# hahnicity/deepards

Measured on AMD Instinct MI355X. Metric: breath-sequences/sec (train step) cnn_linear nb20 seq224, higher is better.
Workload: dtype f32; 1 GPU; cnn_linear+resnet18, synthetic (B=64 per GPU, 20, 1, 224) fp32 train step (BASELINE configs[1]); backbone=resnet18, batch_per_gpu=64, global_batch=64, batch_rule=--batch 64 per rank (weak scaling: the global batch grows with the ranks), n_sub_batches=20, seq_len=224, optimizer=sgd-nesterov+clamp, parallelism=dp1, hipgraph=True

## Files before the change

deepards_amd/csrc/common.h:

```cpp
#pragma once
#include <hip/hip_runtime.h>
#include <stdint.h>

typedef float f32x4 __attribute__((ext_vector_type(4)));
typedef float f32x16 __attribute__((ext_vector_type(16)));

typedef float f32x2v __attribute__((ext_vector_type(2)));
typedef __bf16 bf16x2v __attribute__((ext_vector_type(2)));

#define DA_OK 0
#define DA_EINVAL (-1)

__device__ __forceinline__ int xcd_chunked(int id, int total) {
  const int q = total >> 3, r = total & 7;
  const int xcd = id & 7, s = id >> 3;
  return (xcd < r ? xcd * (q + 1) : r * (q + 1) + (xcd - r) * q) + s;
}

__device__ __forceinline__ uint32_t mix32(uint32_t a, uint32_t b) {
  uint32_t h = a * 0x9E3779B1u ^ (b + 0x7F4A7C15u);
  h ^= h >> 16; h *= 0x85EBCA6Bu;
  h ^= h >> 13; h *= 0xC2B2AE35u;
  h ^= h >> 16;
  return h;
// ... 349 lines not shown
static inline int wgrad_pre_grid(WgradPreTable& pre, int blocks, bool front = false) {
  if (pre.nblocks == 0) return blocks;
  pre.own = front ? -1 : (blocks + 7) & ~7;
  return (front ? blocks : pre.own) + pre.nblocks;
}

struct WgradChain {
  WgradPreTable pre, next;
  int pre_job[WGRAD_PRE_MAX], next_job[WGRAD_PRE_MAX];
  float* const* dws;
  int* reduced;
};
static inline void wgrad_chain_init(WgradChain* c, float* const* dws, int accumulate, int* reduced) {
  c->pre.n = c->pre.nblocks = c->pre.own = 0;
  c->pre.first_block[0] = 0;
  c->pre.accumulate = accumulate;
  c->next = c->pre;
  c->dws = dws;
  c->reduced = reduced;
}
static inline void wgrad_chain_offer(WgradChain* c, int job, const da_wgrad_job& j, int splits) {
  if (!c || !c->dws || !c->dws[job] || c->next.n >= WGRAD_PRE_MAX) return;
  WgradPreTable& t = c->next;
  t.d[t.n] = {j.workspace, c->dws[job], splits, j.ntaps, j.N, j.C};
  c->next_job[t.n] = job;
  t.first_block[t.n + 1] = t.first_block[t.n] + (j.ntaps * j.N * j.C + 1023) / 1024;
  ++t.n;
  t.nblocks = (t.first_block[t.n] + 7) & ~7;
}
static inline WgradPreTable wgrad_chain_take(WgradChain* c) {
  WgradPreTable t;
  t.n = t.nblocks = t.accumulate = t.own = 0;
  t.first_block[0] = 0;
  if (!c) return t;
  t = c->pre;
  for (int i = 0; i < t.n; ++i) c->reduced[c->pre_job[i]] = 1;
  c->pre = c->next;
  for (int i = 0; i < c->next.n; ++i) c->pre_job[i] = c->next_job[i];
  c->next.n = c->next.nblocks = 0;
  return t;
}

struct WgradPlan {
  int tn, tc;
  int splits;
  int kchunk;
};
int wgrad_plan_jobs(const da_wgrad_job* jobs, int n, int chained, WgradPlan* plan);

bool wino_wgrad_eligible(const da_wgrad_job& j);
void wino_wgrad_plan_jobs(const da_wgrad_job* jobs, int n, int chained, WgradPlan* plan);
int wino_wgrad_launch(const da_wgrad_job* jobs, const WgradPlan* plan, int n, hipStream_t stream, WgradChain* chain);
void wino4_wgrad_plan(int rows, int L, int* splits, int* qchunk);
int wino4_wgrad_launch(const da_wgrad_job* jobs, const WgradPlan* plan, int n, hipStream_t stream, WgradChain* chain);

bool bf16_wgrad_eligible(const da_wgrad_job& j);
void bf16_wgrad_plan(int rows, int L, int* splits, int* pchunk);
int bf16_wgrad_launch(const da_wgrad_job* jobs, const WgradPlan* plan, int n, int code, hipStream_t stream);

typedef struct {
  const float* x;
  const float* w;
  float* y;
  int rows, Lm, Lsrc, ldx, C, Ldst, ldy, N, dst_stride, dst_off, src_stride, ntaps;
  int src_off[3];
  int wtap[3];
  int accumulate;
  const float* x2;
  const float* w2;
  int tap_split;
} da_conv_job;

extern "C" int da_sizeof_wgrad_reduce_desc(void);
extern "C" int da_sizeof_bn_running_desc(void);
extern "C" int da_sizeof_bn_pgrad_desc(void);
```

deepards_amd/csrc/conv_gemm.hip:

```cpp
#include "common.h"
#include <algorithm>
#include <utility>
#include <vector>

#ifndef WGRAD_GLOAD_AT
#define WGRAD_GLOAD_AT 8
#endif
#ifndef GLOAD_AT
#define GLOAD_AT 3
#endif

struct ConvGemmArgs {
  const float* x;
  const float* w;
  const float* x2;
  const float* w2;
  int tap_split;
  float* y;
  int M, Lsrc, ldx, C;
  int Ldst, ldy, N;
  int dst_stride, dst_off, src_stride;
  int ntaps, so0, so1, so2, wt0, wt1, wt2;
  int accumulate;
  FastDiv divLm;
// ... 1111 lines not shown
  int n_xf = 0;
  for (int i = 0; i < n; ++i) {
    const da_wgrad_job& j = jobs[i];
    if (!j.dy || !j.x || j.ntaps < 1 || j.ntaps > 3 || j.C % 32 || j.N % 32 || j.lddy % 4 || j.ldx % 4 ||
        (j.winograd == 49 && (j.lddy != j.N || j.ldx != j.C)))
      return DA_EINVAL;
    if ((uint64_t)j.rows * j.Lm * (uint64_t)j.Lm >= 0xffffffffull) return DA_EINVAL;
    if (j.winograd != 0 && j.winograd != 1 && j.winograd != 6 && j.winograd != 16 && j.winograd != 49) return DA_EINVAL;
    if ((j.xform || j.dy_half) && (j.winograd || j.src_stride != 1 || j.dy_stride != 1 || j.dy_off || j.Lm != j.Lx ||
                                   (j.dy_half && j.ntaps != 1)))
      return DA_EINVAL;
    if (j.dy_half && !j.xform) return DA_EINVAL;
    if (j.xform && (j.xform != 1 || !j.mean || !j.invstd || !j.gamma || !j.beta || j.Wn < 1 || j.ldstat < j.C || j.ldstat % 4 ||
                    j.Wn < 32 || (uint64_t)j.rows * j.Lm * (uint64_t)j.Wn >= 0xffffffffull))
      return DA_EINVAL;
    if (j.dy_half && (j.Lm & 1 || j.Ldy * 2 != j.Lm)) return DA_EINVAL;
    if (g_act_bf16 && j.winograd != 16) return DA_EINVAL;
    if (j.winograd == 16 || j.winograd == 49 ? !bf16_wgrad_eligible(j) : (j.winograd && !wino_wgrad_eligible(j))) return DA_EINVAL;
    n_xf += (j.xform || j.dy_half) ? 1 : 0;
  }
  const int tgt = (chained && g_wgrad_any && n_xf >= 8) ? (2560 / n_xf < 96 ? 96 : 2560 / n_xf) : 0;
  for (int i = 0; i < n; ++i) {
    const da_wgrad_job& j = jobs[i];
    plan[i].tn = plan[i].tc = 64;
    if (j.winograd == 16 || j.winograd == 49) bf16_wgrad_plan(j.rows, j.Lm, &plan[i].splits, &plan[i].kchunk);
    else if (j.winograd == 6) wino4_wgrad_plan(j.rows, j.Lm, &plan[i].splits, &plan[i].kchunk);
    else if (j.winograd == 0) {
      plan[i] = wgrad_plan(j.rows * j.Lm, j.N, j.C, j.ntaps, (j.xform || j.dy_half) ? tgt : 0);
      if (!plan[i].tn) return DA_EINVAL;
    }
  }
  wino_wgrad_plan_jobs(jobs, n, chained, plan);
  return DA_OK;
}

static void conv_gemm_fill(ConvGemmArgs& g, const da_conv_job& j) {
  g.x = j.x; g.w = j.w; g.y = j.y;
  g.x2 = j.x2 ? j.x2 : j.x; g.w2 = j.w2 ? j.w2 : j.w; g.tap_split = j.x2 ? j.tap_split : 3;
  g.M = j.rows * j.Lm; g.Lsrc = j.Lsrc; g.ldx = j.ldx; g.C = j.C;
  g.Ldst = j.Ldst; g.ldy = j.ldy; g.N = j.N;
  g.dst_stride = j.dst_stride; g.dst_off = j.dst_off; g.src_stride = j.src_stride;
  g.ntaps = j.ntaps;
  g.so0 = j.src_off[0]; g.so1 = j.ntaps > 1 ? j.src_off[1] : 0; g.so2 = j.ntaps > 2 ? j.src_off[2] : 0;
  g.wt0 = j.wtap[0]; g.wt1 = j.ntaps > 1 ? j.wtap[1] : 0; g.wt2 = j.ntaps > 2 ? j.wtap[2] : 0;
  g.accumulate = j.accumulate;
  g.divLm = make_fastdiv((uint32_t)j.Lm);
}

extern "C" {

int da_debug_set(int key, int value) {
  if (key == 3) g_use_tail = value;
  else if (key == 7) g_wgrad_any = value;
  else return DA_EINVAL;
  return DA_OK;
}

int da_conv_gemm(const float* x, const float* w, float* y, int rows, int Lm, int Lsrc, int ldx, int C, int Ldst,
                 int ldy, int N, int dst_stride, int dst_off, int src_stride, int ntaps, const int* src_off,
                 const int* wtap, int accumulate, hipStream_t stream) {
  DA_ENTER();
  if (g_act_bf16) return DA_EINVAL;
  if (!x || !w || !y || rows < 0 || Lm < 1 || ntaps < 1 || ntaps > 3) return DA_EINVAL;
  da_conv_job j = {};
  j.x = x; j.w = w; j.y = y;
  j.rows = rows; j.Lm = Lm; j.Lsrc = Lsrc; j.ldx = ldx; j.C = C; j.Ldst = Ldst; j.ldy = ldy; j.N = N;
  j.dst_stride = dst_stride; j.dst_off = dst_off; j.src_stride = src_stride; j.ntaps = ntaps; j.accumulate = accumulate;
  for (int t = 0; t < ntaps; ++t) {
    j.src_off[t] = src_off[t];
    j.wtap[t] = wtap[t];
  }
  ConvGemmArgs a;
  conv_gemm_fill(a, j);
  return conv_gemm_dispatch(a, stream);
}

int da_conv_gemm_multi(const da_conv_job* jobs, int n, hipStream_t stream) {
  DA_ENTER();
  if (g_act_bf16) return DA_EINVAL;
  if (n < 1 || n > 4 || !jobs) return DA_EINVAL;
  ConvGemmArgs a[4];
  for (int i = 0; i < n; ++i) {
    const da_conv_job& j = jobs[i];
    if (!j.x || !j.w || !j.y || j.rows < 0 || j.Lm < 1 || j.ntaps < 1 || j.ntaps > 3 || j.C % 32 || j.N % 64 || j.ldx % 4)
      return DA_EINVAL;
    if ((uint64_t)j.rows * j.Lm * (uint64_t)j.Lm >= 0xffffffffull) return DA_EINVAL;
    if (j.x2 && (!j.w2 || j.tap_split < 1 || j.tap_split >= j.ntaps)) return DA_EINVAL;
    conv_gemm_fill(a[i], j);
  }
  return launch_conv_multi(a, n, stream);
}

int da_conv1x1_bn(const float* x, int ldx, const float* w, float* y, int ldy, int rows, int R, int Lin, int C, int N, int pool,
                  float* mean, float* invstd, int ldstat, const float* gamma, const float* beta, const float* pend, int pend_c0,
                  long pend_units, int pend_Wu, float eps, float* out_part, hipStream_t stream) {
  DA_ENTER();
  if (g_act_bf16) return DA_EINVAL;
  if (!x || !w || !y || !mean || !invstd || !gamma || !beta || rows < 0 || R < 1 || rows % R || Lin < 1) return DA_EINVAL;
  if (C % 32 || C < 32 || C > 2048 || N % 64 || N < 64 || ldx % 4 || ldx < C || ldy < N || ldstat % 4 || ldstat < C) return DA_EINVAL;
  if (pool && (Lin & 1)) return DA_EINVAL;
  if (rows == 0) return DA_OK;
  const int Lout = pool ? Lin / 2 : Lin;
  const long M = (long)rows * Lout;
  if ((long)R * Lout < 64) return DA_EINVAL;
  if ((uint64_t)rows * Lin * (uint64_t)(ldx > ldy ? ldx : ldy) >= 0x7fffffffull) return DA_EINVAL;
  if ((uint64_t)M * (uint64_t)(R * Lout) >= 0xffffffffull) return DA_EINVAL;
// ... 233 lines not shown
```

deepards_amd/csrc/conv_wino.hip:

```cpp
#include "common.h"
#include <type_traits>

struct WinoArgs {
  const float* x;
  const float* u;
  float* y;
  int MP, L, PL, ldx, C, ldy, N, accumulate;
  FastDiv divPL;
  const long long* drop_seed;
  uint32_t drop_salt;
  float drop_p;
  float* stat_part;
  int stat_Wu;
  const float* in_pend;
  float* in_mean;
  float* in_invstd;
  const float* in_gamma;
  const float* in_beta;
  int in_tiles, in_Wu;
  float in_eps;
};

__device__ __forceinline__ int wino_row(int i) {
  return (i >= 4 && i < 12) ? 2 * (i - 4) : (i < 4 ? 2 * i + 1 : 2 * (i - 12) + 9);
// ... 444 lines not shown
        }
    }
  }

  if (MINI) {
    __syncthreads();
    f32x4* red = reinterpret_cast<f32x4*>(lds);
    if (khalf == 1) {
#pragma unroll
      for (int j = 0; j < 6; ++j)
#pragma unroll
        for (int nt = 0; nt < 2; ++nt) red[((wp * 6 + j) * 2 + nt) * 64 + lane] = acc[j][nt];
    }
    __syncthreads();
    if (khalf == 1) return;
#pragma unroll
    for (int j = 0; j < 6; ++j)
#pragma unroll
      for (int nt = 0; nt < 2; ++nt) {
        const f32x4 o = red[((wp * 6 + j) * 2 + nt) * 64 + lane];
#pragma unroll
        for (int e = 0; e < 4; ++e) acc[j][nt][e] += o[e];
      }
  }

#pragma unroll
  for (int r = 0; r < 4; ++r) {
    const int Q = Q0 + wp * 16 + wino_row(g * 4 + r);
    if (Q >= a.MP) continue;
    const uint32_t rr = fdiv((uint32_t)Q, a.divPL);
    const int i = Q - (int)rr * QL;
    const int nvalid = a.L - 4 * i;
    float* yp = a.y + ((size_t)rr * a.L + 4 * i) * a.ldy + n_blk + prow;
#pragma unroll
    for (int nt = 0; nt < 2; ++nt) {
      const float m0 = acc[0][nt][r], m1 = acc[1][nt][r], m2 = acc[2][nt][r], m3 = acc[3][nt][r], m4 = acc[4][nt][r],
                  m5 = acc[5][nt][r];
      const float sa = m1 + m2, da = m1 - m2, sb = m3 + m4, db = m3 - m4;
      float yv[4] = {m0 + sa + sb, fmaf(2.f, db, da), fmaf(4.f, sb, sa), fmaf(8.f, db, da) + m5};
      float* q0 = yp + nt * 16;
#pragma unroll
      for (int s = 0; s < 4; ++s) {
        if (s < nvalid) {
          float v = yv[s];
          if (a.accumulate) v += q0[(size_t)s * a.ldy];
          q0[(size_t)s * a.ldy] = v;
        }
      }
    }
  }
}

#define W4K_PITCH 20
#define W4K_LDS_FLOATS ((4 * 64 + 2) * W4K_PITCH + 6 * 32 * W4K_PITCH)

template <bool MINI>
__device__ __forceinline__ void conv3_wino4k_body(const WinoArgs& a, const int tile, const int sub, float* lds) {
  constexpr int PITCH = W4K_PITCH, QUADS = MINI ? 32 : 64;
  float* Ph0 = lds;
  float* Ph1 = Ph0 + (QUADS + 1) * PITCH;
  float* Ph2 = Ph1 + QUADS * PITCH;
  float* Ph3 = Ph2 + QUADS * PITCH;
  float* Us = Ph3 + (QUADS + 1) * PITCH;

  const int tid = threadIdx.x, lane = tid & 63, wave = tid >> 6;
  const int ntn = a.N >> 5;
  const int Q0 = (tile / ntn) * 64 + (MINI ? 32 * sub : 0), n_blk = (tile % ntn) * 32;
  const int lm = tid >> 3;
  const int lr = (lm >> 2) * 8 + (lm & 3) + 4 * ((tid >> 2) & 1), lq = tid & 3;
  const int QL = a.PL;

  constexpr int NP = MINI ? 2 : 4, NA = NP + 1;
  int aoff[NA];
  bool aok[NA];
#pragma unroll
  for (int p = 0; p < NA; ++p) {
    const bool extra = p == NA - 1;
    const int idx = p * 64 + lr;
    const int phase = extra ? (((tid >> 2) & 1) ? 3 : 0) : idx / QUADS;
    const int e = extra ? (phase == 0 ? QUADS : -1) : idx % QUADS;
    const int Q = Q0 + e;
    bool ok = Q >= 0 && Q < a.MP && (!extra || tid < 8);
    const uint32_t r = fdiv((uint32_t)(ok ? Q : 0), a.divPL);
    const int i = (ok ? Q : 0) - (int)r * QL;
    const int pos = 4 * i + phase;
    ok = ok && pos < a.L;
    aoff[p] = ((int)r * a.L + (ok ? pos : 0)) * a.ldx + lq * 4;
    aok[p] = ok;
  }
  const float* ub[3];
#pragma unroll
  for (int p = 0; p < 3; ++p) {
    const int idx = p * 64 + lr;
    const int nrow = n_blk + (idx & 31);
    ub[p] = a.u + (size_t)(idx >> 5) * a.N * a.C + (size_t)nrow * a.C + lq * 4;
  }

  f32x4 ra[NA], rb[3];
  auto gload_a = [&](int ks) {
    const int c0 = ks << 4;
#pragma unroll
    for (int p = 0; p < NA; ++p) {
      f32x4 v = {0.f, 0.f, 0.f, 0.f};
      if (aok[p]) v = *reinterpret_cast<const f32x4*>(a.x + aoff[p] + c0);
      ra[p] = v;
    }
  };
  auto gload_b = [&](int ks) {
    const int c0 = ks << 4;
#pragma unroll
    for (int p = 0; p < 3; ++p) rb[p] = *reinterpret_cast<const f32x4*>(ub[p] + c0);
  };

  const int prow = wino_row(lane & 15), g = lane >> 4;
  const int col = (((g & 1) << 1) | (g >> 1)) * 4;
  const int wp = MINI ? (wave & 1) : wave, khalf = wave >> 1;
  const int pr = wp * 16 + prow;
  const int Q_lane = Q0 + pr;
  const int Qc = Q_lane < a.MP ? Q_lane : 0;
  const int i_lane = Qc - (int)fdiv((uint32_t)Qc, a.divPL) * QL;
// ... 47 lines not shown
        for (int e = 0; e < 4; ++e)
          acc[j][nt] = __builtin_amdgcn_mfma_f32_16x16x4f32(D[j][e], uf[e], acc[j][nt], 0, 0, 0);
      }
  }

  if (MINI) {
    __syncthreads();
    f32x4* red = reinterpret_cast<f32x4*>(lds);
    if (khalf == 1) {
#pragma unroll
      for (int j = 0; j < 6; ++j)
#pragma unroll
        for (int nt = 0; nt < 2; ++nt) red[((wp * 6 + j) * 2 + nt) * 64 + lane] = acc[j][nt];
    }
    __syncthreads();
    if (khalf == 1) return;
#pragma unroll
    for (int j = 0; j < 6; ++j)
#pragma unroll
      for (int nt = 0; nt < 2; ++nt) {
        const f32x4 o = red[((wp * 6 + j) * 2 + nt) * 64 + lane];
#pragma unroll
        for (int e = 0; e < 4; ++e) acc[j][nt][e] += o[e];
      }
  }

#pragma unroll
  for (int r = 0; r < 4; ++r) {
    const int Q = Q0 + wp * 16 + wino_row(g * 4 + r);
    if (Q >= a.MP) continue;
    const uint32_t rr = fdiv((uint32_t)Q, a.divPL);
    const int i = Q - (int)rr * QL;
    const int nvalid = a.L - 4 * i;
    float* yp = a.y + ((size_t)rr * a.L + 4 * i) * a.ldy + n_blk + prow;
#pragma unroll
    for (int nt = 0; nt < 2; ++nt) {
      const float m0 = acc[0][nt][r], m1 = acc[1][nt][r], m2 = acc[2][nt][r], m3 = acc[3][nt][r], m4 = acc[4][nt][r],
                  m5 = acc[5][nt][r];
      const float sa = m1 + m2, da = m1 - m2, sb = m3 + m4, db = m3 - m4;
      float yv[4] = {m0 + sa + sb, fmaf(2.f, db, da), fmaf(4.f, sb, sa), fmaf(8.f, db, da) + m5};
      float* q0 = yp + nt * 16;
#pragma unroll
      for (int s = 0; s < 4; ++s) {
        if (s < nvalid) {
          float v = yv[s];
          if (a.accumulate) v += q0[(size_t)s * a.ldy];
          q0[(size_t)s * a.ldy] = v;
        }
      }
    }
  }
}

__global__ __launch_bounds__(256, 3) void conv3_wino4k_kernel(WinoArgs a, int nmini, int nmini_pad, int full) {
  __shared__ float lds[W4K_LDS_FLOATS];
  if ((int)blockIdx.x < nmini_pad) {
    if ((int)blockIdx.x < nmini) conv3_wino4k_body<true>(a, full + ((int)blockIdx.x >> 1), blockIdx.x & 1, lds);
    return;
  }
  conv3_wino4k_body<false>(a, xcd_chunked(blockIdx.x - nmini_pad, full), 0, lds);
}

__global__ __launch_bounds__(256) void conv3_wino4_kernel(WinoArgs a, int nmini, int nmini_pad, int full) {
  __shared__ float lds[W4_LDS_FLOATS];
  if ((int)blockIdx.x < nmini_pad) {
    if ((int)blockIdx.x < nmini) conv3_wino4_body<true>(a, full + ((int)blockIdx.x >> 1), blockIdx.x & 1, lds);
    return;
  }
  conv3_wino4_body<false>(a, xcd_chunked(blockIdx.x - nmini_pad, full), 0, lds);
}

static int g_wino_tail = 1;
static int g_wino4_k16 = 1;

struct WinoWgradArgs {
  const float* dy;
  const float* x;
  float* slab;
  int MP, L, PL, lddy, N, ldx, C, pchunk;
  FastDiv divPL;
};

#ifndef WW_KP
#define WW_KP 32
#endif
#ifndef WW_MIN_WAVES
#define WW_MIN_WAVES 4
#define WW_UNROLL 8
#endif
#define WW_LDS_FLOATS ((2 * WW_KP + 2 * (WW_KP + 2)) * 64)

__device__ __forceinline__ void wino_wgrad_body(const WinoWgradArgs& a, const int block_id, const int nblocks, float* lds) {
  constexpr int KP = WW_KP, NRB = KP / 16;
  float* YE = lds;
  float* YO = lds + KP * 64;
  float* XE = lds + 2 * KP * 64;
  float* XO = XE + (KP + 2) * 64;

  const int tid = threadIdx.x, lane = tid & 63, wave = tid >> 6;
  const int wm = wave >> 1, wn = wave & 1;
  const int ntc = a.C >> 6, tiles = (a.N >> 6) * ntc;
  const int lin = xcd_chunked(block_id, nblocks);
  const int bx = lin % tiles, split = lin / tiles;
  const int n_blk = (bx / ntc) * 64, c_blk = (bx % ntc) * 64;
  const int PL = a.PL;
  const int k_beg = split * a.pchunk, k_end = min(a.MP, k_beg + a.pchunk);

  const int lrow = tid >> 4, lq = tid & 15;
  f32x4 ry[2 * NRB], rx[2 * NRB + 1];
  auto gload = [&](int k0) {
#pragma unroll
    for (int rb = 0; rb < NRB; ++rb) {
      const int P = k0 + lrow + 16 * rb;
      const bool ok = P < a.MP;
      const uint32_t r = fdiv((uint32_t)(ok ? P : 0), a.divPL);
      const int i = (ok ? P : 0) - (int)r * PL;
      const size_t pos = (size_t)r * a.L + 2 * i;
      const bool ok1 = ok && 2 * i + 1 < a.L;
      const bool okk = ok && P < k_end;
      f32x4 z = {0.f, 0.f, 0.f, 0.f};
      ry[2 * rb] = okk ? *reinterpret_cast<const f32x4*>(a.dy + pos * a.lddy + n_blk + lq * 4) : z;
      ry[2 * rb + 1] = (okk && ok1) ? *reinterpret_cast<const f32x4*>(a.dy + (pos + 1) * a.lddy + n_blk + lq * 4) : z;
      rx[2 * rb] = ok ? *reinterpret_cast<const f32x4*>(a.x + pos * a.ldx + c_blk + lq * 4) : z;
      rx[2 * rb + 1] = ok1 ? *reinterpret_cast<const f32x4*>(a.x + (pos + 1) * a.ldx + c_blk + lq * 4) : z;
    }
    if (tid < 32) {
// ... 22 lines not shown
    for (int rb = 0; rb < NRB; ++rb) {
      const int row = lrow + 16 * rb;
      *reinterpret_cast<f32x4*>(&YE[row * 64 + lq * 4]) = ry[2 * rb];
      *reinterpret_cast<f32x4*>(&YO[row * 64 + lq * 4]) = ry[2 * rb + 1];
      *reinterpret_cast<f32x4*>(&XE[(row + 1) * 64 + lq * 4]) = rx[2 * rb];
      *reinterpret_cast<f32x4*>(&XO[(row + 1) * 64 + lq * 4]) = rx[2 * rb + 1];
    }
    if (tid < 16) *reinterpret_cast<f32x4*>(&XO[lq * 4]) = rx[2 * NRB];
    else if (tid < 32) *reinterpret_cast<f32x4*>(&XE[(KP + 1) * 64 + lq * 4]) = rx[2 * NRB];
    const int Pm = k0 + (lane & 31);
    const int im = Pm - (int)fdiv((uint32_t)(Pm < a.MP ? Pm : 0), a.divPL) * PL;
    const uint32_t fmask = (uint32_t)__ballot(Pm < a.MP && im == 0);
    const uint32_t lmask = (uint32_t)__ballot(Pm < a.MP && im == PL - 1);
    __syncthreads();
#pragma unroll WW_UNROLL
    for (int kk = 0; kk < KP / 2; ++kk) {
      if (kk == KP / 4) {
        __builtin_amdgcn_sched_barrier(0);
        if (k0 + KP < k_end) gload(k0 + KP);
        __builtin_amdgcn_sched_barrier(0);
      }
      const int p = 2 * kk + fh;
      const float y0 = YE[p * 64 + wm * 32 + frow], y1 = YO[p * 64 + wm * 32 + frow];
      float d0 = XO[p * 64 + wn * 32 + frow];
      const float d1 = XE[(p + 1) * 64 + wn * 32 + frow], d2 = XO[(p + 1) * 64 + wn * 32 + frow];
      float d3 = XE[(p + 2) * 64 + wn * 32 + frow];
      if ((fmask >> p) & 1) d0 = 0.f;
      if ((lmask >> p) & 1) d3 = 0.f;
      acc[0] = __builtin_amdgcn_mfma_f32_32x32x2f32(y0, d0 - d2, acc[0], 0, 0, 0);
      acc[1] = __builtin_amdgcn_mfma_f32_32x32x2f32(y0 + y1, d1 + d2, acc[1], 0, 0, 0);
      acc[2] = __builtin_amdgcn_mfma_f32_32x32x2f32(y0 - y1, d2 - d1, acc[2], 0, 0, 0);
      acc[3] = __builtin_amdgcn_mfma_f32_32x32x2f32(y1, d1 - d3, acc[3], 0, 0, 0);
    }
  }

  float* out = a.slab + (size_t)split * 3 * a.N * a.C;
  const size_t plane = (size_t)a.N * a.C;
#pragma unroll
  for (int r = 0; r < 16; ++r) {
    const int n = n_blk + wm * 32 + (r & 3) + 8 * (r >> 2) + 4 * fh;
    const int c = c_blk + wn * 32 + frow;
    const float h = 0.5f * (acc[1][r] + acc[2][r]);
    float* o = out + (size_t)n * a.C + c;
    o[0] = acc[0][r] + h;
    o[plane] = 0.5f * (acc[1][r] - acc[2][r]);
    o[2 * plane] = h - acc[3][r];
  }
}

struct WinoWgradTable {
  WinoWgradArgs d[24];
  int first_block[25];
  int n;
};
static_assert(sizeof(WinoWgradTable) + sizeof(WgradPreTable) <= 4096, "kernel arguments: 4 KB");

__global__ __launch_bounds__(256, WW_MIN_WAVES) void wino_wgrad_multi_kernel(WinoWgradTable t, WgradPreTable pre) {
  __shared__ float lds[WW_LDS_FLOATS];
  const int b = wgrad_pre_dispatch(pre);
  if (b < 0 || b >= t.first_block[t.n]) return;
  int i = 0;
  while (i + 1 < t.n && b >= t.first_block[i + 1]) ++i;
  wino_wgrad_body(t.d[i], b - t.first_block[i], t.first_block[i + 1] - t.first_block[i], lds);
}

bool wino_wgrad_eligible(const da_wgrad_job& j) {
  return j.ntaps == 3 && j.dy_stride == 1 && j.dy_off == 0 && j.src_stride == 1 && j.src_off[0] == -1 &&
         j.src_off[1] == 0 && j.src_off[2] == 1 && j.Lm == j.Ldy && j.Lm == j.Lx && j.N % 64 == 0 && j.C % 64 == 0 &&
         j.N >= 64 && j.C >= 64;
}

#ifndef WW_PCHUNK
#define WW_PCHUNK 640
#endif

static void wino_wgrad_plan(int rows, int L, int* splits, int* pchunk, int f) {
  const int MP = rows * ((L + 1) / 2);
  const int base = WW_PCHUNK / (f > 1 ? f : 1) >= 32 ? WW_PCHUNK / (f > 1 ? f : 1) : 32;
  int sp = (MP + base - 1) / base;
  if (sp < 1) sp = 1;
  int pc = ((MP + sp - 1) / sp + 31) / 32 * 32;
  if (pc < 32) pc = 32;
  *splits = (MP + pc - 1) / pc > 0 ? (MP + pc - 1) / pc : 1;
  *pchunk = pc;
}

void wino_wgrad_plan_jobs(const da_wgrad_job* jobs, int n, int chained, WgradPlan* plan) {
  constexpr int SLOTS = 1024;
  long total = 0;
  int njobs = 0;
  for (int i = 0; i < n; ++i) {
    if (jobs[i].winograd != 1) continue;
    plan[i].tn = plan[i].tc = 64;
    wino_wgrad_plan(jobs[i].rows, jobs[i].Lm, &plan[i].splits, &plan[i].kchunk, 1);
    total += (long)(jobs[i].N / 64) * (jobs[i].C / 64) * plan[i].splits;
    ++njobs;
  }
  if (!chained || njobs > 24 || total <= SLOTS || total % SLOTS == 0) return;
  const long full = total / SLOTS * SLOTS;
  long cum = 0;
  for (int i = 0; i < n; ++i) {
    if (jobs[i].winograd != 1) continue;
    cum += (long)(jobs[i].N / 64) * (jobs[i].C / 64) * plan[i].splits;
    if (cum > full) wino_wgrad_plan(jobs[i].rows, jobs[i].Lm, &plan[i].splits, &plan[i].kchunk, 2);
  }
}

int wino_wgrad_launch(const da_wgrad_job* jobs, const WgradPlan* plan, int n, hipStream_t s, WgradChain* chain) {
  WinoWgradTable t;
  int cnt = 0, blocks = 0;
  auto flush = [&]() -> int {
    if (!cnt) return DA_OK;
    t.n = cnt;
    t.first_block[cnt] = blocks;
    WgradPreTable pre = wgrad_chain_take(chain);
    hipLaunchKernelGGL(wino_wgrad_multi_kernel, dim3(wgrad_pre_grid(pre, blocks)), dim3(256), 0, s, t, pre);
    DA_CHECK_LAUNCH();
    cnt = 0;
    blocks = 0;
    return DA_OK;
  };
  for (int i = 0; i < n; ++i) {
    const da_wgrad_job& j = jobs[i];
    if (j.winograd != 1) continue;
    WinoWgradArgs& a = t.d[cnt];
    a.dy = j.dy; a.x = j.x; a.slab = j.workspace;
    a.L = j.Lm; a.PL = (j.Lm + 1) / 2; a.MP = j.rows * a.PL;
    a.lddy = j.lddy; a.N = j.N; a.ldx = j.ldx; a.C = j.C; a.pchunk = plan[i].kchunk;
    a.divPL = make_fastdiv((uint32_t)a.PL);
    t.first_block[cnt] = blocks;
    blocks += (j.N / 64) * (j.C / 64) * plan[i].splits;
    wgrad_chain_offer(chain, i, j, plan[i].splits);
    if (++cnt == 24) {
      int rc = flush();
      if (rc) return rc;
    }
  }
  return flush();
}

#ifndef WW4_KQ
#define WW4_KQ 16
#endif
#ifndef WW4_MIN_WAVES
#define WW4_MIN_WAVES 3
#endif
#ifndef WW4_UNROLL
#define WW4_UNROLL 4
#endif
#define WW4_LDS_FLOATS ((4 * WW4_KQ + 4 * WW4_KQ + 2) * 64)

__device__ __forceinline__ void wino4_wgrad_body(const WinoWgradArgs& a, const int block_id, const int nblocks, float* lds) {
  constexpr int KQ = WW4_KQ, NRB = KQ / 16;
  float* Y = lds;
  float* X0 = lds + 4 * KQ * 64;
  float* X1 = X0 + (KQ + 1) * 64;
  float* X2 = X1 + KQ * 64;
  float* X3 = X2 + KQ * 64;

  const int tid = threadIdx.x, lane = tid & 63, wave = tid >> 6;
  const int wm = wave >> 1, wn = wave & 1;
  const int ntc = a.C >> 6, tiles = (a.N >> 6) * ntc;
  const int lin = xcd_chunked(block_id, nblocks);
  const int bx = lin % tiles, split = lin / tiles;
  const int n_blk = (bx / ntc) * 64, c_blk = (bx % ntc) * 64;
  const int QL = a.PL;
  const int k_beg = split * a.pchunk, k_end = min(a.MP, k_beg + a.pchunk);

  const int lrow = tid >> 4, lq = tid & 15;
  f32x4 ry[4 * NRB], rx[4 * NRB + 1];
  auto gload = [&](int k0) {
    const f32x4 z = {0.f, 0.f, 0.f, 0.f};
#pragma unroll
    for (int rb = 0; rb < NRB; ++rb) {
      const int Q = k0 + lrow + 16 * rb;
      const bool ok = Q < a.MP;
      const uint32_t r = fdiv((uint32_t)(ok ? Q : 0), a.divPL);
      const int i = (ok ? Q : 0) - (int)r * QL;
      const size_t pos = (size_t)r * a.L + 4 * i;
      const bool okk = ok && Q < k_end;
#pragma unroll
      for (int ph = 0; ph < 4; ++ph) {
        const bool in = 4 * i + ph < a.L;
        ry[4 * rb + ph] = (okk && in) ? *reinterpret_cast<const f32x4*>(a.dy + (pos + ph) * a.lddy + n_blk + lq * 4) : z;
        rx[4 * rb + ph] = (ok && in) ? *reinterpret_cast<const f32x4*>(a.x + (pos + ph) * a.ldx + c_blk + lq * 4) : z;
      }
    }
    if (tid < 32) {
      const int Qh = tid < 16 ? k0 - 1 : k0 + KQ;
      const bool okh = Qh >= 0 && Qh < a.MP;
      const uint32_t rh = fdiv((uint32_t)(okh ? Qh : 0), a.divPL);
      const int ih = (okh ? Qh : 0) - (int)rh * QL;
      const int pp = 4 * ih + (tid < 16 ? 3 : 0);
      f32x4 v = z;
      if (okh && pp < a.L) v = *reinterpret_cast<const f32x4*>(a.x + ((size_t)rh * a.L + pp) * a.ldx + c_blk + lq * 4);
      rx[4 * NRB] = v;
    }
  };

  f32x16 acc[6];
#pragma unroll
  for (int j = 0; j < 6; ++j)
#pragma unroll
    for (int r = 0; r < 16; ++r) acc[j][r] = 0.f;

  const int frow = lane & 31, fh = lane >> 5;
  if (k_beg < k_end) gload(k_beg);
  for (int k0 = k_beg; k0 < k_end; k0 += KQ) {
    __syncthreads();
#pragma unroll
    for (int rb = 0; rb < NRB; ++rb) {
      const int row = lrow + 16 * rb;
#pragma unroll
      for (int ph = 0; ph < 4; ++ph) *reinterpret_cast<f32x4*>(&Y[(ph * KQ + row) * 64 + lq * 4]) = ry[4 * rb + ph];
      *reinterpret_cast<f32x4*>(&X0[row * 64 + lq * 4]) = rx[4 * rb];
      *reinterpret_cast<f32x4*>(&X1[row * 64 + lq * 4]) = rx[4 * rb + 1];
      *reinterpret_cast<f32x4*>(&X2[row * 64 + lq * 4]) = rx[4 * rb + 2];
      *reinterpret_cast<f32x4*>(&X3[(row + 1) * 64 + lq * 4]) = rx[4 * rb + 3];
    }
    if (tid < 16) *reinterpret_cast<f32x4*>(&X3[lq * 4]) = rx[4 * NRB];
    else if (tid < 32) *reinterpret_cast<f32x4*>(&X0[KQ * 64 + lq * 4]) = rx[4 * NRB];
    const int Qm = k0 + (lane & (KQ - 1));
    const int im = Qm - (int)fdiv((uint32_t)(Qm < a.MP ? Qm : 0), a.divPL) * QL;
    const uint32_t fmask = (uint32_t)__ballot(Qm < a.MP && im == 0);
    const uint32_t lmask = (uint32_t)__ballot(Qm < a.MP && im == QL - 1);
    __syncthreads();
#pragma unroll WW4_UNROLL
    for (int kk = 0; kk < KQ / 2; ++kk) {
      if (kk == KQ / 4) {
        __builtin_amdgcn_sched_barrier(0);
        if (k0 + KQ < k_end) gload(k0 + KQ);
        __builtin_amdgcn_sched_barrier(0);
      }
      const int p = 2 * kk + fh;
      const int yo = p * 64 + wm * 32 + frow, xo = p * 64 + wn * 32 + frow;
      const float y0 = Y[yo], y1 = Y[KQ * 64 + yo], y2 = Y[2 * KQ * 64 + yo], y3 = Y[3 * KQ * 64 + yo];
      float d0 = X3[xo];
      const float d1 = X0[xo], d2 = X1[xo], d3 = X2[xo], d4 = X3[xo + 64];
      float d5 = X0[xo + 64];
      if ((fmask >> p) & 1) d0 = 0.f;
      if ((lmask >> p) & 1) d5 = 0.f;
      const float ya = y0 + y2, yb = y1 + y3, yc = fmaf(4.f, y2, y0), yd = 2.f * fmaf(4.f, y3, y1);
      const float e1 = fmaf(-4.f, d2, d4), e2 = fmaf(-4.f, d1, d3), f1 = d4 - d2, f2 = d3 - d1;
      acc[0] = __builtin_amdgcn_mfma_f32_32x32x2f32(y0, fmaf(4.f, d0, fmaf(-5.f, d2, d4)), acc[0], 0, 0, 0);
      acc[1] = __builtin_amdgcn_mfma_f32_32x32x2f32(ya + yb, e1 + e2, acc[1], 0, 0, 0);
      acc[2] = __builtin_amdgcn_mfma_f32_32x32x2f32(ya - yb, e1 - e2, acc[2], 0, 0, 0);
      acc[3] = __builtin_amdgcn_mfma_f32_32x32x2f32(yc + yd, fmaf(2.f, f2, f1), acc[3], 0, 0, 0);
      acc[4] = __builtin_amdgcn_mfma_f32_32x32x2f32(yc - yd, fmaf(-2.f, f2, f1), acc[4], 0, 0, 0);
      acc[5] = __builtin_amdgcn_mfma_f32_32x32x2f32(y3, fmaf(4.f, d1, fmaf(-5.f, d3, d5)), acc[5], 0, 0, 0);
    }
  }

  float* out = a.slab + (size_t)split * 3 * a.N * a.C;
  const size_t plane = (size_t)a.N * a.C;
#pragma unroll
  for (int r = 0; r < 16; ++r) {
    const int n = n_blk + wm * 32 + (r & 3) + 8 * (r >> 2) + 4 * fh;
    const int c = c_blk + wn * 32 + frow;
    const float s12 = acc[1][r] + acc[2][r], s34 = acc[3][r] + acc[4][r];
    float* o = out + (size_t)n * a.C + c;
    o[0] = fmaf(0.25f, acc[0][r], fmaf(1.0f / 24.0f, s34, -(1.0f / 6.0f) * s12));
    o[plane] = fmaf(1.0f / 6.0f, acc[2][r] - acc[1][r], (1.0f / 12.0f) * (acc[3][r] - acc[4][r]));
    o[2 * plane] = fmaf(1.0f / 6.0f, s34 - s12, acc[5][r]);
  }
}

__global__ __launch_bounds__(256, WW4_MIN_WAVES) void wino4_wgrad_multi_kernel(WinoWgradTable t, WgradPreTable pre) {
  __shared__ float lds[WW4_LDS_FLOATS];
  const int b = wgrad_pre_dispatch(pre);
  if (b < 0 || b >= t.first_block[t.n]) return;
  int i = 0;
  while (i + 1 < t.n && b >= t.first_block[i + 1]) ++i;
  wino4_wgrad_body(t.d[i], b - t.first_block[i], t.first_block[i + 1] - t.first_block[i], lds);
}

#ifndef WW4_QCHUNK
#define WW4_QCHUNK 320
#endif

void wino4_wgrad_plan(int rows, int L, int* splits, int* qchunk) {
  const int MQ = rows * ((L + 3) / 4);
  int sp = (MQ + WW4_QCHUNK - 1) / WW4_QCHUNK;
  if (sp < 1) sp = 1;
  int qc = ((MQ + sp - 1) / sp + WW4_KQ - 1) / WW4_KQ * WW4_KQ;
  if (qc < WW4_KQ) qc = WW4_KQ;
  *splits = (MQ + qc - 1) / qc > 0 ? (MQ + qc - 1) / qc : 1;
  *qchunk = qc;
}

int wino4_wgrad_launch(const da_wgrad_job* jobs, const WgradPlan* plan, int n, hipStream_t s, WgradChain* chain) {
  WinoWgradTable t;
  int cnt = 0, blocks = 0;
  auto flush = [&]() -> int {
    if (!cnt) return DA_OK;
    t.n = cnt;
    t.first_block[cnt] = blocks;
    WgradPreTable pre = wgrad_chain_take(chain);
    hipLaunchKernelGGL(wino4_wgrad_multi_kernel, dim3(wgrad_pre_grid(pre, blocks)), dim3(256), 0, s, t, pre);
    DA_CHECK_LAUNCH();
    cnt = 0;
    blocks = 0;
    return DA_OK;
  };
  for (int i = 0; i < n; ++i) {
    const da_wgrad_job& j = jobs[i];
    if (j.winograd != 6) continue;
    WinoWgradArgs& a = t.d[cnt];
    a.dy = j.dy; a.x = j.x; a.slab = j.workspace;
    a.L = j.Lm; a.PL = (j.Lm + 3) / 4; a.MP = j.rows * a.PL;
    a.lddy = j.lddy; a.N = j.N; a.ldx = j.ldx; a.C = j.C; a.pchunk = plan[i].kchunk;
    a.divPL = make_fastdiv((uint32_t)a.PL);
    t.first_block[cnt] = blocks;
    blocks += (j.N / 64) * (j.C / 64) * plan[i].splits;
    wgrad_chain_offer(chain, i, j, plan[i].splits);
    if (++cnt == 24) {
      int rc = flush();
      if (rc) return rc;
    }
  }
  return flush();
}

__global__ __launch_bounds__(256) void wino_weight_kernel(const float* __restrict__ w, float* __restrict__ u, int co,
                                                          int ci, int transpose) {
  const int N = transpose ? ci : co, C = transpose ? co : ci;
  const size_t total = (size_t)N * C;
  const size_t idx = (size_t)blockIdx.x * blockDim.x + threadIdx.x;
  if (idx >= total) return;
  const int n = (int)(idx / C), c = (int)(idx - (size_t)n * C);
  const float* src = transpose ? w + ((size_t)c * ci + n) * 3 : w + ((size_t)n * ci + c) * 3;
  const float g0 = transpose ? src[2] : src[0], g1 = src[1], g2 = transpose ? src[0] : src[2];
  u[idx] = g0;
  u[total + idx] = (g0 + g1 + g2) * 0.5f;
  u[2 * total + idx] = (g0 - g1 + g2) * 0.5f;
  u[3 * total + idx] = g2;
}

__global__ __launch_bounds__(256) void wino4_weight_kernel(const float* __restrict__ w, float* __restrict__ u, int co,
                                                           int ci, int transpose) {
  const int N = transpose ? ci : co, C = transpose ? co : ci;
  const size_t total = (size_t)N * C;
  const size_t idx = (size_t)blockIdx.x * blockDim.x + threadIdx.x;
  if (idx >= total) return;
  const int n = (int)(idx / C), c = (int)(idx - (size_t)n * C);
  const float* src = transpose ? w + ((size_t)c * ci + n) * 3 : w + ((size_t)n * ci + c) * 3;
  const float g0 = transpose ? src[2] : src[0], g1 = src[1], g2 = transpose ? src[0] : src[2];
  wino4_taps(g0, g1, g2, u + idx, total);
}

extern "C" {

int da_wino4_weights(const float* w, float* u, int co, int ci, int transpose, hipStream_t stream) {
  DA_ENTER();
  if (!w || !u || co < 1 || ci < 1) return DA_EINVAL;
  const size_t total = (size_t)co * ci;
  hipLaunchKernelGGL(wino4_weight_kernel, dim3((unsigned)((total + 255) / 256)), dim3(256), 0, stream, w, u, co, ci,
                     transpose);
  DA_CHECK_LAUNCH();
  return DA_OK;
}

struct WinoBnIn {
  const float* pend; float* mean; float* invstd; const float* gamma; const float* beta; float eps;
};

static int conv3_winograd_impl(const float* x, const float* u, float* y, int rows, int L, int ldx, int C, int ldy, int N,
                               int accumulate, const long long* drop_seed, unsigned drop_salt, float drop_p, float* stat_part,
                               int stat_R, hipStream_t stream, const WinoBnIn* bn = nullptr, int outs = 2) {
  DA_ENTER();
  if (g_act_bf16) return DA_EINVAL;
  if (outs == 4 && (stat_part || bn || drop_p > 0.f)) return DA_EINVAL;
  if (!x || !u || !y || rows < 0 || L < 1 || C % 32 || N % 32 || C < 32 || N < 32 || ldx % 4 || ldx < C || ldy < N)
    return DA_EINVAL;
  if (rows == 0) return DA_OK;
  if ((uint64_t)rows * L * (uint64_t)(ldx > ldy ? ldx : ldy) >= 0x7fffffffull) return DA_EINVAL;
  WinoArgs a;
  a.x = x; a.u = u; a.y = y;
  a.L = L; a.PL = (L + outs - 1) / outs; a.MP = rows * a.PL;
  a.ldx = ldx; a.C = C; a.ldy = ldy; a.N = N; a.accumulate = accumulate;
  a.drop_seed = drop_seed; a.drop_salt = drop_salt; a.drop_p = drop_p;
  a.stat_part = stat_part; a.stat_Wu = (stat_part || bn) ? stat_R * a.PL : 1;
  if ((stat_part || bn) && (stat_R < 1 || rows % stat_R || a.stat_Wu < 64 || accumulate)) return DA_EINVAL;
  a.in_pend = nullptr; a.in_mean = a.in_invstd = nullptr; a.in_gamma = a.in_beta = nullptr; a.in_tiles = 0; a.in_Wu = 1; a.in_eps = 0.f;
  if (bn) {
    if (!bn->pend || !bn->mean || !bn->invstd || !bn->gamma || !bn->beta || C > 128 || ldx != C) return DA_EINVAL;
    a.in_pend = bn->pend; a.in_mean = bn->mean; a.in_invstd = bn->invstd; a.in_gamma = bn->gamma; a.in_beta = bn->beta;
    a.in_eps = bn->eps; a.in_Wu = stat_R * L; a.in_tiles = (int)(((long)rows * L + 63) / 64);
    if (a.in_Wu < 64) return DA_EINVAL;
  }
  a.divPL = make_fastdiv((uint32_t)a.PL);
  if ((uint64_t)a.MP * (uint64_t)a.PL >= 0xffffffffull) return DA_EINVAL;
  const int tiles = ((a.MP + 63) / 64) * (N / 32);
  const int R = tiles % 256;
  int nmini = 0, full = tiles;
  const bool dropping = drop_p > 0.f;
  if (g_wino_tail && !stat_part && !bn && !dropping && tiles > 256 && R >= 1 && R <= 128) {
    nmini = 2 * R;
    full = tiles - R;
  }
  const int nmini_pad = (nmini + 7) / 8 * 8;
  if (outs == 4 && g_wino4_k16)
    hipLaunchKernelGGL(conv3_wino4k_kernel, dim3(nmini_pad + full), dim3(256), 0, stream, a, nmini, nmini_pad, full);
  else if (outs == 4)
    hipLaunchKernelGGL(conv3_wino4_kernel, dim3(nmini_pad + full), dim3(256), 0, stream, a, nmini, nmini_pad, full);
  else if (bn && stat_part) hipLaunchKernelGGL(conv3_wino_bn_kernel<true>, dim3(full), dim3(256), 0, stream, a, full);
  else if (bn) hipLaunchKernelGGL(conv3_wino_bn_kernel<false>, dim3(full), dim3(256), 0, stream, a, full);
  else if (stat_part) hipLaunchKernelGGL(conv3_wino_stats_kernel, dim3(full), dim3(256), 0, stream, a, full);
  else if (dropping) hipLaunchKernelGGL(conv3_wino_drop_kernel, dim3(full), dim3(256), 0, stream, a, full);
  else hipLaunchKernelGGL(conv3_wino_kernel, dim3(nmini_pad + full), dim3(256), 0, stream, a, nmini, nmini_pad, full);
  DA_CHECK_LAUNCH();
  return DA_OK;
}

int da_conv3_winograd(const float* x, const float* u, float* y, int rows, int L, int ldx, int C, int ldy, int N,
                      int accumulate, hipStream_t stream) {
  return conv3_winograd_impl(x, u, y, rows, L, ldx, C, ldy, N, accumulate, nullptr, 0u, 0.f, nullptr, 0, stream);
}

int da_conv3_winograd4(const float* x, const float* u, float* y, int rows, int L, int ldx, int C, int ldy, int N,
                       int accumulate, hipStream_t stream) {
  return conv3_winograd_impl(x, u, y, rows, L, ldx, C, ldy, N, accumulate, nullptr, 0u, 0.f, nullptr, 0, stream, nullptr, 4);
}

int da_conv3_winograd_drop(const float* x, const float* u, float* y, int rows, int L, int ldx, int C, int ldy, int N,
                           const long long* drop_seed, unsigned drop_salt, float drop_p, float* stat_part, int R,
                           hipStream_t stream) {
  if (drop_p < 0.f || drop_p >= 1.f || (drop_p > 0.f && !drop_seed)) return DA_EINVAL;
  return conv3_winograd_impl(x, u, y, rows, L, ldx, C, ldy, N, 0, drop_seed, drop_salt, drop_p, stat_part, R, stream);
}

int da_conv3_winograd_bn(const float* x, const float* u, float* y, int rows, int L, int C, int ldy, int N, int R,
                         const float* in_pend, float* in_mean, float* in_invstd, const float* gamma, const float* beta,
                         float eps, const long long* drop_seed, unsigned drop_salt, float drop_p, float* stat_part,
                         hipStream_t stream) {
  if (drop_p < 0.f || drop_p >= 1.f || (drop_p > 0.f && !drop_seed)) return DA_EINVAL;
  WinoBnIn bn = {in_pend, in_mean, in_invstd, gamma, beta, eps};
  return conv3_winograd_impl(x, u, y, rows, L, C, C, ldy, N, 0, drop_seed, drop_salt, drop_p, stat_part, R, stream, &bn);
}

size_t da_stat_records_floats(long units, int N) {
  const size_t tiles = (size_t)((units + 63) / 64);
  return tiles * 4 * (size_t)N + tiles * 2;
}

int da_wino_debug_tail(int on) {
  if (on & ~1) {
    g_wino4_k16 = on & 1;
    return DA_OK;
  }
  g_wino_tail = on;
  return DA_OK;
}

int da_wino_weights(const float* w, float* u, int co, int ci, int transpose, hipStream_t stream) {
  DA_ENTER();
// ... 10 lines not shown
```

Baseline: 452,000 breath-sequences/s.

## Skip the dead sixth Winograd output row when a sequence spans two tiles

Adds a specialised F(4,3) Winograd path for sequences whose length needs exactly two output quads and is not a multiple of four (e.g. L=7). In the forward conv, one block now handles both quads of a row together, shares the overlapping input, and computes only 5 of the 6 transform rows for the second quad, which outputs at most 3 values. The weight-grad kernel gets a SKIP5 variant that computes the sixth product once per pair of K steps instead of every step, with a smaller unroll. Both paths are on by default and can be turned off through a debug key. The new index mapping and partial-quad handling add complexity and risk of wrong outputs at boundaries.

```diff
diff --git a/deepards_amd/csrc/common.h b/deepards_amd/csrc/common.h
--- a/deepards_amd/csrc/common.h
+++ b/deepards_amd/csrc/common.h
@@ -425,6 +425,7 @@
 void wino_wgrad_plan_jobs(const da_wgrad_job* jobs, int n, int chained, WgradPlan* plan);
 int wino_wgrad_launch(const da_wgrad_job* jobs, const WgradPlan* plan, int n, hipStream_t stream, WgradChain* chain);
 void wino4_wgrad_plan(int rows, int L, int* splits, int* qchunk);
+extern int g_wino4_skip5;
 int wino4_wgrad_launch(const da_wgrad_job* jobs, const WgradPlan* plan, int n, hipStream_t stream, WgradChain* chain);
 
 bool bf16_wgrad_eligible(const da_wgrad_job& j);
diff --git a/deepards_amd/csrc/conv_gemm.hip b/deepards_amd/csrc/conv_gemm.hip
--- a/deepards_amd/csrc/conv_gemm.hip
+++ b/deepards_amd/csrc/conv_gemm.hip
@@ -1187,6 +1187,7 @@
 int da_debug_set(int key, int value) {
   if (key == 3) g_use_tail = value;
   else if (key == 7) g_wgrad_any = value;
+  else if (key == 11) g_wino4_skip5 = value;
   else return DA_EINVAL;
   return DA_OK;
 }
diff --git a/deepards_amd/csrc/conv_wino.hip b/deepards_amd/csrc/conv_wino.hip
--- a/deepards_amd/csrc/conv_wino.hip
+++ b/deepards_amd/csrc/conv_wino.hip
@@ -520,11 +520,12 @@
 }
 
 #define W4K_PITCH 20
-#define W4K_LDS_FLOATS ((4 * 64 + 2) * W4K_PITCH + 6 * 32 * W4K_PITCH)
+#define W4K_TILE_QUADS 64
+#define W4K_LDS_FLOATS ((4 * W4K_TILE_QUADS + 2) * W4K_PITCH + 6 * 32 * W4K_PITCH)
 
 template <bool MINI>
 __device__ __forceinline__ void conv3_wino4k_body(const WinoArgs& a, const int tile, const int sub, float* lds) {
-  constexpr int PITCH = W4K_PITCH, QUADS = MINI ? 32 : 64;
+  constexpr int PITCH = W4K_PITCH, QUADS = MINI ? W4K_TILE_QUADS / 2 : W4K_TILE_QUADS;
   float* Ph0 = lds;
   float* Ph1 = Ph0 + (QUADS + 1) * PITCH;
   float* Ph2 = Ph1 + QUADS * PITCH;
@@ -533,7 +534,7 @@
 
   const int tid = threadIdx.x, lane = tid & 63, wave = tid >> 6;
   const int ntn = a.N >> 5;
-  const int Q0 = (tile / ntn) * 64 + (MINI ? 32 * sub : 0), n_blk = (tile % ntn) * 32;
+  const int Q0 = (tile / ntn) * W4K_TILE_QUADS + (MINI ? W4K_TILE_QUADS / 2 * sub : 0), n_blk = (tile % ntn) * 32;
   const int lm = tid >> 3;
   const int lr = (lm >> 2) * 8 + (lm & 3) + 4 * ((tid >> 2) & 1), lq = tid & 3;
   const int QL = a.PL;
@@ -687,13 +688,183 @@
   }
 }
 
+template <bool MINI>
+__device__ __forceinline__ void conv3_wino4k_skip5_body(const WinoArgs& a, const int tile, const int sub, float* lds) {
+  constexpr int PITCH = W4K_PITCH, QUADS = MINI ? W4K_TILE_QUADS / 2 : W4K_TILE_QUADS, HALF = QUADS / 2;
+  float* Ph0 = lds;
+  float* Ph1 = Ph0 + QUADS * PITCH;
+  float* Ph2 = Ph1 + QUADS * PITCH;
+  float* Ph3 = Ph2 + QUADS * PITCH;
+  float* Us = Ph3 + QUADS * PITCH;
+
+  const int tid = threadIdx.x, lane = tid & 63, wave = tid >> 6;
+  const int ntn = a.N >> 5;
+  const int Q0 = (tile / ntn) * W4K_TILE_QUADS + (MINI ? W4K_TILE_QUADS / 2 * sub : 0), n_blk = (tile % ntn) * 32;
+  const int lm = tid >> 3;
+  const int lr = (lm >> 2) * 8 + (lm & 3) + 4 * ((tid >> 2) & 1), lq = tid & 3;
+
+  constexpr int NP = MINI ? 2 : 4;
+  int aoff[NP];
+  bool aok[NP];
+#pragma unroll
+  for (int p = 0; p < NP; ++p) {
+    const int idx = p * 64 + lr;
+    const int phase = idx / QUADS, e = idx % QUADS;
+    const int second = e >= HALF ? 1 : 0;
+    const int Q = Q0 + 2 * (e - second * HALF) + second;
+    const int pos = 4 * second + phase;
+    const bool ok = Q < a.MP && pos < a.L;
+    aoff[p] = ok ? ((Q >> 1) * a.L + pos) * a.ldx + lq * 4 : 0;
+    aok[p] = ok;
+  }
+  const float* ub[3];
+#pragma unroll
+  for (int p = 0; p < 3; ++p) {
+    const int idx = p * 64 + lr;
+    const int nrow = n_blk + (idx & 31);
+    ub[p] = a.u + (size_t)(idx >> 5) * a.N * a.C + (size_t)nrow * a.C + lq * 4;
+  }
+
+  f32x4 ra[NP], rb[3];
+  auto gload_a = [&](int ks) {
+    const int c0 = ks << 4;
+#pragma unroll
+    for (int p = 0; p < NP; ++p) {
+      f32x4 v = {0.f, 0.f, 0.f, 0.f};
+      if (aok[p]) v = *reinterpret_cast<const f32x4*>(a.x + aoff[p] + c0);
+      ra[p] = v;
+    }
+  };
+  auto gload_b = [&](int ks) {
+    const int c0 = ks << 4;
+#pragma unroll
+    for (int p = 0; p < 3; ++p) rb[p] = *reinterpret_cast<const f32x4*>(ub[p] + c0);
+  };
+
+  const int prow = wino_row(lane & 15), g = lane >> 4;
+  const int col = (((g & 1) << 1) | (g >> 1)) * 4;
+  const int nh = wave & 1;
+  const int qh = MINI ? 0 : wave >> 1, khalf = wave >> 1;
+  const int rF = (qh * 16 + prow) * PITCH + col, rS = rF + HALF * PITCH;
+
+  f32x4 accF[6], accS[5];
+#pragma unroll
+  for (int j = 0; j < 6; ++j) accF[j] = f32x4{0.f, 0.f, 0.f, 0.f};
+#pragma unroll
+  for (int j = 0; j < 5; ++j) accS[j] = f32x4{0.f, 0.f, 0.f, 0.f};
+
+  const int kc = a.C >> 4;
+  gload_a(0);
+  gload_b(0);
+  for (int ks = 0; ks < kc; ++ks) {
+    __syncthreads();
+#pragma unroll
+    for (int p = 0; p < NP; ++p) {
+      const int idx = p * 64 + lr;
+      const int phase = idx / QUADS, e = idx % QUADS;
+      float* panel = phase == 0 ? Ph0 : (phase == 1 ? Ph1 : (phase == 2 ? Ph2 : Ph3));
+      *reinterpret_cast<f32x4*>(&panel[e * PITCH + lq * 4]) = ra[p];
+    }
+#pragma unroll
+    for (int p = 0; p < 3; ++p) *reinterpret_cast<f32x4*>(&Us[(p * 64 + lr) * PITCH + lq * 4]) = rb[p];
+    __syncthreads();
+    __builtin_amdgcn_sched_barrier(0);
+    if (ks + 1 < kc) {
+      gload_b(ks + 1);
+      gload_a(ks + 1);
+    }
+    __builtin_amdgcn_sched_barrier(0);
+    if (MINI && (ks & 1) != khalf) continue;
+    const f32x4 z = {0.f, 0.f, 0.f, 0.f};
+    const f32x4 f1 = *reinterpret_cast<const f32x4*>(&Ph0[rF]), f2 = *reinterpret_cast<const f32x4*>(&Ph1[rF]);
+    const f32x4 f3 = *reinterpret_cast<const f32x4*>(&Ph2[rF]), f4 = *reinterpret_cast<const f32x4*>(&Ph3[rF]);
+    const f32x4 s1 = *reinterpret_cast<const f32x4*>(&Ph0[rS]), s2 = *reinterpret_cast<const f32x4*>(&Ph1[rS]);
+    const f32x4 s3 = *reinterpret_cast<const f32x4*>(&Ph2[rS]), s4 = *reinterpret_cast<const f32x4*>(&Ph3[rS]);
+    f32x4 DF[6], DS[6];
+    wino4_input_transform(z, f1, f2, f3, f4, s1, DF);
+    wino4_input_transform(f4, s1, s2, s3, s4, z, DS);
+#pragma unroll
+    for (int j = 0; j < 6; ++j) {
+      const f32x4 uf = *reinterpret_cast<const f32x4*>(&Us[(j * 32 + nh * 16 + prow) * PITCH + col]);
+#pragma unroll
+      for (int e = 0; e < 4; ++e) {
+        accF[j] = __builtin_amdgcn_mfma_f32_16x16x4f32(DF[j][e], uf[e], accF[j], 0, 0, 0);
+        if (j < 5) accS[j] = __builtin_amdgcn_mfma_f32_16x16x4f32(DS[j][e], uf[e], accS[j], 0, 0, 0);
+      }
+    }
+  }
+
+  if (MINI) {
+    __syncthreads();
+    f32x4* red = reinterpret_cast<f32x4*>(lds);
+    if (khalf == 1) {
+#pragma unroll
+      for (int j = 0; j < 6; ++j) red[(nh * 11 + j) * 64 + lane] = accF[j];
+#pragma unroll
+      for (int j = 0; j < 5; ++j) red[(nh * 11 + 6 + j) * 64 + lane] = accS[j];
+    }
+    __syncthreads();
+    if (khalf == 1) return;
+#pragma unroll
+    for (int j = 0; j < 6; ++j) {
+      const f32x4 o = red[(nh * 11 + j) * 64 + lane];
+#pragma unroll
+      for (int e = 0; e < 4; ++e) accF[j][e] += o[e];
+    }
+#pragma unroll
+    for (int j = 0; j < 5; ++j) {
+      const f32x4 o = red[(nh * 11 + 6 + j) * 64 + lane];
+#pragma unroll
+      for (int e = 0; e < 4; ++e) accS[j][e] += o[e];
+    }
+  }
+
+  const int nS = a.L - 4;
+#pragma unroll
+  for (int r = 0; r < 4; ++r) {
+    const int Q = Q0 + 2 * (qh * 16 + wino_row(g * 4 + r));
+    if (Q >= a.MP) continue;
+    float* yp = a.y + (size_t)(Q >> 1) * a.L * a.ldy + n_blk + nh * 16 + prow;
+    {
+      const float m0 = accF[0][r], m1 = accF[1][r], m2 = accF[2][r], m3 = accF[3][r], m4 = accF[4][r], m5 = accF[5][r];
+      const float sa = m1 + m2, da = m1 - m2, sb = m3 + m4, db = m3 - m4;
+      const float yv[4] = {m0 + sa + sb, fmaf(2.f, db, da), fmaf(4.f, sb, sa), fmaf(8.f, db, da) + m5};
+#pragma unroll
+      for (int s = 0; s < 4; ++s) {
+        float v = yv[s];
+        if (a.accumulate) v += yp[(size_t)s * a.ldy];
+        yp[(size_t)s * a.ldy] = v;
+      }
+    }
+    {
+      const float m0 = accS[0][r], m1 = accS[1][r], m2 = accS[2][r], m3 = accS[3][r], m4 = accS[4][r];
+      const float sa = m1 + m2, da = m1 - m2, sb = m3 + m4, db = m3 - m4;
+      const float yv[3] = {m0 + sa + sb, fmaf(2.f, db, da), fmaf(4.f, sb, sa)};
+      float* q1 = yp + (size_t)4 * a.ldy;
+#pragma unroll
+      for (int s = 0; s < 3; ++s) {
+        if (s < nS) {
+          float v = yv[s];
+          if (a.accumulate) v += q1[(size_t)s * a.ldy];
+          q1[(size_t)s * a.ldy] = v;
+        }
+      }
+    }
+  }
+}
+
+template <bool SKIP5>
 __global__ __launch_bounds__(256, 3) void conv3_wino4k_kernel(WinoArgs a, int nmini, int nmini_pad, int full) {
   __shared__ float lds[W4K_LDS_FLOATS];
   if ((int)blockIdx.x < nmini_pad) {
-    if ((int)blockIdx.x < nmini) conv3_wino4k_body<true>(a, full + ((int)blockIdx.x >> 1), blockIdx.x & 1, lds);
+    if ((int)blockIdx.x < nmini) {
+      if (SKIP5) conv3_wino4k_skip5_body<true>(a, full + ((int)blockIdx.x >> 1), blockIdx.x & 1, lds);
+      else conv3_wino4k_body<true>(a, full + ((int)blockIdx.x >> 1), blockIdx.x & 1, lds);
+    }
     return;
   }
-  conv3_wino4k_body<false>(a, xcd_chunked(blockIdx.x - nmini_pad, full), 0, lds);
+  if (SKIP5) conv3_wino4k_skip5_body<false>(a, xcd_chunked(blockIdx.x - nmini_pad, full), 0, lds);
+  else conv3_wino4k_body<false>(a, xcd_chunked(blockIdx.x - nmini_pad, full), 0, lds);
 }
 
 __global__ __launch_bounds__(256) void conv3_wino4_kernel(WinoArgs a, int nmini, int nmini_pad, int full) {
@@ -707,6 +878,9 @@
 
 static int g_wino_tail = 1;
 static int g_wino4_k16 = 1;
+int g_wino4_skip5 = 1;
+
+static bool wino4_skip5_applies(int L, int QL) { return g_wino4_skip5 && QL == 2 && (L & 3) != 0; }
 
 struct WinoWgradArgs {
   const float* dy;
@@ -835,6 +1009,7 @@
   WinoWgradArgs d[24];
   int first_block[25];
   int n;
+  int skip5;
 };
 static_assert(sizeof(WinoWgradTable) + sizeof(WgradPreTable) <= 4096, "kernel arguments: 4 KB");
 
@@ -895,6 +1070,7 @@
   auto flush = [&]() -> int {
     if (!cnt) return DA_OK;
     t.n = cnt;
+    t.skip5 = 0;
     t.first_block[cnt] = blocks;
     WgradPreTable pre = wgrad_chain_take(chain);
     hipLaunchKernelGGL(wino_wgrad_multi_kernel, dim3(wgrad_pre_grid(pre, blocks)), dim3(256), 0, s, t, pre);
@@ -931,8 +1107,12 @@
 #ifndef WW4_UNROLL
 #define WW4_UNROLL 4
 #endif
+#ifndef WW4_SKIP5_UNROLL
+#define WW4_SKIP5_UNROLL 2
+#endif
 #define WW4_LDS_FLOATS ((4 * WW4_KQ + 4 * WW4_KQ + 2) * 64)
 
+template <bool SKIP5>
 __device__ __forceinline__ void wino4_wgrad_body(const WinoWgradArgs& a, const int block_id, const int nblocks, float* lds) {
   constexpr int KQ = WW4_KQ, NRB = KQ / 16;
   float* Y = lds;
@@ -1008,9 +1188,14 @@
     const uint32_t fmask = (uint32_t)__ballot(Qm < a.MP && im == 0);
     const uint32_t lmask = (uint32_t)__ballot(Qm < a.MP && im == QL - 1);
     __syncthreads();
-#pragma unroll WW4_UNROLL
-    for (int kk = 0; kk < KQ / 2; ++kk) {
-      if (kk == KQ / 4) {
+    constexpr int UNR = SKIP5 ? WW4_SKIP5_UNROLL : WW4_UNROLL, UNR2 = UNR / 2;
+    static_assert(UNR % 2 == 0 && KQ % 8 == 0, "the K loop is unrolled in whole pairs of kk");
+#pragma unroll UNR2
+    for (int k2 = 0; k2 < KQ / 4; ++k2)
+#pragma unroll
+    for (int u = 0; u < 2; ++u) {
+      const int kk = 2 * k2 + u;
+      if (u == 0 && k2 == KQ / 8) {
         __builtin_amdgcn_sched_barrier(0);
         if (k0 + KQ < k_end) gload(k0 + KQ);
         __builtin_amdgcn_sched_barrier(0);
@@ -1030,7 +1215,15 @@
       acc[2] = __builtin_amdgcn_mfma_f32_32x32x2f32(ya - yb, e1 - e2, acc[2], 0, 0, 0);
       acc[3] = __builtin_amdgcn_mfma_f32_32x32x2f32(yc + yd, fmaf(2.f, f2, f1), acc[3], 0, 0, 0);
       acc[4] = __builtin_amdgcn_mfma_f32_32x32x2f32(yc - yd, fmaf(-2.f, f2, f1), acc[4], 0, 0, 0);
-      acc[5] = __builtin_amdgcn_mfma_f32_32x32x2f32(y3, fmaf(4.f, d1, fmaf(-5.f, d3, d5)), acc[5], 0, 0, 0);
+      if (!SKIP5) {
+        acc[5] = __builtin_amdgcn_mfma_f32_32x32x2f32(y3, fmaf(4.f, d1, fmaf(-5.f, d3, d5)), acc[5], 0, 0, 0);
+      } else if (u == 0) {
+        const int p5 = 2 * kk + 2 * fh;
+        const int y5o = p5 * 64 + wm * 32 + frow, x5o = p5 * 64 + wn * 32 + frow;
+        const float g3 = Y[3 * KQ * 64 + y5o];
+        const float g1 = X0[x5o], g2 = X2[x5o], g5 = X0[x5o + 64];
+        acc[5] = __builtin_amdgcn_mfma_f32_32x32x2f32(g3, fmaf(4.f, g1, fmaf(-5.f, g2, g5)), acc[5], 0, 0, 0);
+      }
     }
   }
 
@@ -1054,7 +1247,9 @@
   if (b < 0 || b >= t.first_block[t.n]) return;
   int i = 0;
   while (i + 1 < t.n && b >= t.first_block[i + 1]) ++i;
-  wino4_wgrad_body(t.d[i], b - t.first_block[i], t.first_block[i + 1] - t.first_block[i], lds);
+  const bool skip5 = t.skip5 && t.d[i].PL == 2 && (t.d[i].L & 3) != 0;
+  if (skip5) wino4_wgrad_body<true>(t.d[i], b - t.first_block[i], t.first_block[i + 1] - t.first_block[i], lds);
+  else wino4_wgrad_body<false>(t.d[i], b - t.first_block[i], t.first_block[i + 1] - t.first_block[i], lds);
 }
 
 #ifndef WW4_QCHUNK
@@ -1079,6 +1274,7 @@
     t.n = cnt;
     t.first_block[cnt] = blocks;
     WgradPreTable pre = wgrad_chain_take(chain);
+    t.skip5 = g_wino4_skip5 != 0;
     hipLaunchKernelGGL(wino4_wgrad_multi_kernel, dim3(wgrad_pre_grid(pre, blocks)), dim3(256), 0, s, t, pre);
     DA_CHECK_LAUNCH();
     cnt = 0;
@@ -1092,6 +1288,8 @@
     a.dy = j.dy; a.x = j.x; a.slab = j.workspace;
     a.L = j.Lm; a.PL = (j.Lm + 3) / 4; a.MP = j.rows * a.PL;
     a.lddy = j.lddy; a.N = j.N; a.ldx = j.ldx; a.C = j.C; a.pchunk = plan[i].kchunk;
+    static_assert(WW4_KQ % 8 == 0, "skip5: K steps start at even quads");
+    if (a.pchunk % WW4_KQ) return DA_EINVAL;
     a.divPL = make_fastdiv((uint32_t)a.PL);
     t.first_block[cnt] = blocks;
     blocks += (j.N / 64) * (j.C / 64) * plan[i].splits;
@@ -1182,8 +1380,11 @@
     full = tiles - R;
   }
   const int nmini_pad = (nmini + 7) / 8 * 8;
-  if (outs == 4 && g_wino4_k16)
-    hipLaunchKernelGGL(conv3_wino4k_kernel, dim3(nmini_pad + full), dim3(256), 0, stream, a, nmini, nmini_pad, full);
+  static_assert(W4K_TILE_QUADS == 64, "skip5: a wave owns 16 rows = 32 quads; full and half tiles start at even quads");
+  if (outs == 4 && g_wino4_k16 && wino4_skip5_applies(L, a.PL))
+    hipLaunchKernelGGL(conv3_wino4k_kernel<true>, dim3(nmini_pad + full), dim3(256), 0, stream, a, nmini, nmini_pad, full);
+  else if (outs == 4 && g_wino4_k16)
+    hipLaunchKernelGGL(conv3_wino4k_kernel<false>, dim3(nmini_pad + full), dim3(256), 0, stream, a, nmini, nmini_pad, full);
   else if (outs == 4)
     hipLaunchKernelGGL(conv3_wino4_kernel, dim3(nmini_pad + full), dim3(256), 0, stream, a, nmini, nmini_pad, full);
   else if (bn && stat_part) hipLaunchKernelGGL(conv3_wino_bn_kernel<true>, dim3(full), dim3(256), 0, stream, a, full);
```

After: 456,600 breath-sequences/s, median of 6. 1.0% higher.
